# ShadowLive/ExtIO_sddc

Measured on AMD Instinct MI355X. Metric: input MSamples/s at decim=2 + achieved % HBM roofline, 1 GPU; IQ max-rel-err, higher is better.
Workload: dtype f32 (int16 in, complex64 out)

## Files before the change

extio_sddc_amd/csrc/ddc_frame_common.hpp:

```cpp
#pragma once

#include <hip/hip_runtime.h>

#include "ddc_device_io.hpp"
#include "ddc_kernels.h"
#include "fft_device.hpp"

namespace sddc {
namespace {

constexpr int NT = 256;
constexpr int HALF = 4096;
constexpr int HOP = 6144;
constexpr int BLOCK = 65536;
constexpr int FRAMES = 11;

__device__ __forceinline__ int swz(int e) { return e ^ ((e >> 4) & 15); }

template <bool RAND>
__device__ __forceinline__ float derand(int v)
{
    const float f = (float)v;
    if constexpr (!RAND) return f;
    return __int_as_float(__float_as_int(f) ^ (v << 31));
}

template <int DIR>
__device__ __forceinline__ float2 TW(float2 a, float2 w) { return DIR < 0 ? cmul(a, w) : cmulc(a, w); }

__device__ __forceinline__ float2 split_pr(float2 zk, float2 zc, float2 p, float r)
{
    const float vx = fmaf(r, zc.y, zk.x), vy = fmaf(r, zc.x, zk.y);
    return make_float2(fmaf(vx, p.x, -vy * p.y), fmaf(vx, p.y, vy * p.x));
}

template <int N>
__device__ __forceinline__ int emit_base(int k)
{
    return k == 0 ? -N / 4 : N / 2 + (3 * N / 4) * (k - 1);
}

template <int NB, bool NCO, bool CS16>
__device__ __forceinline__ void emit_frame(void *__restrict__ out, int fbase, int k, int t, const float2 (&u)[16],
                                           const OutArgs &oa, const NcoArgs &nco)
{
    const __amdgpu_buffer_rsrc_t ro = buf_rsrc(static_cast<char *>(out) + (size_t)fbase * out_bytes<CS16>());
    const int r0 = k == 0 ? 4 : 0;
#pragma unroll
    for (int r = 0; r < 12; r++) {
        if (r < r0) continue;
        float2 v = flip(u[r], oa.lsbmask);
        if constexpr (NCO) v = nco_mix(v, nco, fbase + t + NB * r);
        store_iq<CS16>(v, ro, (unsigned)t, (unsigned)(NB * r), oa);
    }
}

#define XRD(dst, expr) do { dst = (expr); asm volatile("" ::: "memory"); } while (0)

__device__ __forceinline__ void wave_lds_sync()
{
    __builtin_amdgcn_fence(__ATOMIC_RELEASE, "wavefront");
    __builtin_amdgcn_wave_barrier();
    __builtin_amdgcn_fence(__ATOMIC_ACQUIRE, "wavefront");
}

__device__ __forceinline__ void st_row(float2 *buf, unsigned A, int r, int rstride, float2 v)
{
    *(reinterpret_cast<float2 *>(reinterpret_cast<char *>(buf) + (A ^ (8u * (unsigned)r))) + rstride * r) = v;
}

__device__ __forceinline__ float2 &lds_x(float2 *buf, unsigned lane8, int R)
{
    return *reinterpret_cast<float2 *>(reinterpret_cast<char *>(buf) + (lane8 ^ (8u * (unsigned)swz(R))));
}
#define LX(buf, lane, R) lds_x(buf, 8u * (unsigned)swz(lane), R)


template <int DIR, bool EARLY>
__device__ __forceinline__ void table_twiddle(float2 *a, const float2 *tbl, int S, int j)
{
    if constexpr (EARLY) {
        float2 tw[15];
#pragma unroll
        for (int r = 1; r <= 8; r++) XRD(tw[r - 1], tbl[(r - 1) * S + j]);
#pragma unroll
        for (int r = 1; r <= 8; r++) a[r] = TW<DIR>(a[r], tw[r - 1]);
#pragma unroll
        for (int r = 9; r < 16; r++) XRD(tw[r - 1], tbl[(r - 1) * S + j]);
#pragma unroll
        for (int r = 9; r < 16; r++) a[r] = TW<DIR>(a[r], tw[r - 1]);
    } else {
#pragma unroll
        for (int r = 1; r < 16; r++) {
            float2 w;
            XRD(w, tbl[(r - 1) * S + j]);
            a[r] = TW<DIR>(a[r], w);
        }
    }
}

__device__ __forceinline__ void load_frame(const int *__restrict__ in32, int blk, int k, int (&x)[16])
{
    const __amdgpu_buffer_rsrc_t rs = buf_rsrc(in32 + ((size_t)blk * BLOCK + (size_t)k * HOP) / 2);
    const unsigned vo = 4u * threadIdx.x;
#pragma unroll
    for (int r = 0; r < 16; r++) x[r] = buf_load4<SDDC_LD_AUX>(rs, vo, 4u * NT * r);
}

}
}
```

extio_sddc_amd/csrc/ddc_fs.hip:

```cpp
#include <hip/hip_runtime.h>

#include <type_traits>

#include "ddc_frame_common.hpp"
#include "ddc_queue.hpp"
#include "ddc_stamps.hpp"
#include "ddc_fs_perm.h"
#include "split_coeffs.h"

namespace sddc {
namespace {

#ifdef SDDC_STAMPS
__device__ unsigned g_fs_stamps[2048 * 4 * kStampWords];
#endif

__device__ __forceinline__ float dpp_partner(float v)
{
    return __int_as_float(__builtin_amdgcn_mov_dpp(__float_as_int(v), 0xB1, 0xF, 0xF, true));
}

__device__ __forceinline__ void split_v2(float2 &za, float2 &vb, float2 zb, float ra, float rb)
{
    asm("s_nop 1\n\t"
        "v_fmac_f32_dpp %2, %1, %7 quad_perm:[1,0,3,2] row_mask:0xf bank_mask:0xf\n\t"
        "v_fmac_f32_dpp %3, %0, %7 quad_perm:[1,0,3,2] row_mask:0xf bank_mask:0xf\n\t"
        "v_fmac_f32_dpp %0, %5, %6 quad_perm:[1,0,3,2] row_mask:0xf bank_mask:0xf\n\t"
        "v_fmac_f32_dpp %1, %4, %6 quad_perm:[1,0,3,2] row_mask:0xf bank_mask:0xf"
        : "+v"(za.x), "+v"(za.y), "+&v"(vb.x), "+&v"(vb.y)
        : "v"(zb.x), "v"(zb.y), "v"(ra), "v"(rb));
}

__device__ __forceinline__ void split_v1(float2 &z, float2 zp, float r)
{
    asm("s_nop 1\n\t"
        "v_fmac_f32_dpp %0, %3, %4 quad_perm:[1,0,3,2] row_mask:0xf bank_mask:0xf\n\t"
        "v_fmac_f32_dpp %1, %2, %4 quad_perm:[1,0,3,2] row_mask:0xf bank_mask:0xf"
        : "+v"(z.x), "+v"(z.y)
        : "v"(zp.x), "v"(zp.y), "v"(r));
}

__device__ __forceinline__ float2 p_mul(float2 v, float2 q)
{
    return make_float2(fmaf(v.x, q.x, -v.y * q.y), fmaf(v.x, q.y, v.y * q.x));
}

template <bool LSB>
__device__ __forceinline__ float2 quarter_flip(float2 v, int s)
{
    s &= 3;
    float2 o = s == 0 ? v : s == 1 ? make_float2(v.y, -v.x) : s == 2 ? make_float2(-v.x, -v.y) : make_float2(-v.y, v.x);
    if constexpr (LSB) o.y = -o.y;
    return o;
}

template <int QT, bool LSB, bool NCO, bool CS16>
__device__ __forceinline__ void emit_frame_q(void *__restrict__ out, int fbase, int k, int t, const float2 (&u)[16],
                                             const OutArgs &oa, const NcoArgs &nco)
{
    const __amdgpu_buffer_rsrc_t ro = buf_rsrc(static_cast<char *>(out) + (size_t)fbase * out_bytes<CS16>());
    const int r0 = k == 0 ? 4 : 0;
#pragma unroll
    for (int r = 0; r < 12; r++) {
        if (r < r0) continue;
        float2 v = quarter_flip<LSB>(u[r], QT * r);
        if constexpr (NCO) v = nco_mix(v, nco, fbase + t + NT * r);
        store_iq<CS16>(v, ro, (unsigned)t, (unsigned)(NT * r), oa);
    }
}

constexpr int kQWave = 3;
constexpr int kFsPqAhead = 1;
__device__ __forceinline__ int fs_row_slot(int t) { return 272 * (t >> 4) + (t >= 128) + 34 * ((t & 15) >> 1) + (t & 1); }
__device__ __forceinline__ int fs_pair_row(int t) { return 2 * (t >> 5) + (t & 1); }
__device__ __forceinline__ int fs_pair_col(int t) { return (t >> 1) & 15; }
__device__ __forceinline__ int fs_pair_slot(int t) { return t + 2 * (t >> 5); }
constexpr int kFsLds = 4352;
constexpr int kFsTw = NT + 1;

enum { kSchedStatic = 0, kSchedQueue = 1, kSchedSteal = 2 };
template <int SCHED> struct SchedOf { using T = StealSchedule; };
template <> struct SchedOf<kSchedStatic> { using T = StaticSchedule; };
template <> struct SchedOf<kSchedQueue> { using T = FrameSchedule<1>; };

template <int ZR>
__device__ __forceinline__ constexpr bool zrow(int k) { return zr_row<ZR>(k); }

template <int SCHED, int ZR, bool RAND, bool LSB, bool NCO, bool CS16>
__global__ __launch_bounds__(NT, 4) void r2iq_fs_kernel(
    const int *__restrict__ in32, void *__restrict__ out, int nframes, const float2 *__restrict__ tw_p1,
    const float2 *__restrict__ rec_f, const float4 *__restrict__ pqf, const float2 *__restrict__ fsl, int tunebin,
    OutArgs oa, NcoArgs nco, unsigned *__restrict__ wq, int ns, unsigned slotw, int xmap, int minrem, int pub,
    unsigned *__restrict__ tlog, unsigned ttag, int use_tab, FsShares shares)
{
    __shared__ __attribute__((aligned(16))) float2 lds[kFsLds];
    __shared__ __attribute__((aligned(16))) float2 twl[15 * 16];
    __shared__ __attribute__((aligned(16))) float2 wtab[2 * kFsTw];
    __shared__ int s_next;
    static_assert(sizeof(float2) * (kFsLds + 15 * 16 + 2 * kFsTw) + sizeof(int) <= 163840 / 4,
                  "four workgroups per CU");

    const int tid = (int)threadIdx.x;
    const int w = xmap ? (int)(blockIdx.x & 7u) * (int)(gridDim.x >> 3) + (int)(blockIdx.x >> 3) : (int)blockIdx.x;
    constexpr int QLANE = 64 * kQWave;
    const bool qw = __builtin_amdgcn_readfirstlane(tid >> 6) == kQWave;
    typename SchedOf<SCHED>::T fsch;
    auto split = [&](int G, int v) __attribute__((always_inline)) {
        if constexpr (SCHED == kSchedStatic) return fs_static_split(ns, G, v, slotw, use_tab, shares);
        else return slot_split(ns, G, v, slotw);
    };
    unsigned t_start = 0u;
    if constexpr (SCHED == kSchedStatic)
        if (tlog) t_start = (unsigned)__builtin_amdgcn_s_memrealtime();
    int x[16];
    {
        const int G = (int)gridDim.x, a0 = split(G, w), b0 = split(G, w + 1);
        const int f0s = a0 < b0 ? a0 : -1;
        if (f0s >= 0) load_frame(in32, f0s / FRAMES, f0s % FRAMES, x);
        if (qw) {
            int f0[1];
            if constexpr (SCHED == kSchedSteal) fsch.init(wq, nframes, ns, w, G, slotw, f0, minrem, pub);
            else if constexpr (SCHED == kSchedStatic) fsch.init_range(a0, b0, f0);
            else fsch.init(wq, nframes, ns, w, G, slotw, f0);
            if (tid == QLANE) s_next = f0[0];
        }
        for (int i = tid; i < 15 * 16; i += NT) twl[i] = tw_p1[i];
        wtab[tid + (tid >= 128)] = rec_f[tid];
        wtab[kFsTw + tid + (tid >= 128)] = rec_f[NT + tid];
        __syncthreads();
        const int f = s_next;
        if (f >= 0 && f0s < 0) load_frame(in32, f / FRAMES, f % FRAMES, x);
    }
    int f = s_next;
    int blk = f / FRAMES, k = f - blk * FRAMES;
    const int col_ = kFsPerm[tid];
    const int qt = (tunebin >> 2) & 3;
    const bool w0 = __builtin_amdgcn_readfirstlane(tid >> 6) == 0;
    float cr[16];
    {
        const __amdgpu_buffer_rsrc_t rr = buf_rsrc(reinterpret_cast<const float *>(pqf) + 2 * HALF);
#pragma unroll
        for (int k = 0; k < 16; k++)
            if (!zrow<ZR>(k)) cr[k] = __uint_as_float(__builtin_amdgcn_raw_buffer_load_b32(rr, 4u * tid, 4u * NT * k, 0));
    }
    constexpr int AZR = ZR > 0 ? ZR : -ZR;
    constexpr int CPP = SCHED == kSchedStatic && !NCO && !CS16 && AZR >= 3 ? (AZR >= 4 && AZR <= 7 ? AZR + 1 : AZR) : 0;
    float2 cp[16];
    if constexpr (CPP > 0) {
        const __amdgpu_buffer_rsrc_t rq = buf_rsrc(pqf);
#pragma unroll
        for (int k = 0; k < 16; k++)
            if (!zrow<ZR>(k) && (k < CPP || 15 - k < CPP))
                cp[k] = buf_load8(rq, 16u * tid, 4096u * (k < 8 ? k : 15 - k) + (k < 8 ? 0u : 8u));
    }
    constexpr bool GREG = SCHED == kSchedStatic;
    float2 cg0, cg1, cg4;
    if constexpr (GREG) {
        const __amdgpu_buffer_rsrc_t rfs = buf_rsrc(fsl);
        const unsigned t8 = 8u * (unsigned)tid;
        cg0 = buf_load8(rfs, t8, 0);
        cg1 = buf_load8(rfs, t8, 8u * NT);
        cg4 = buf_load8(rfs, t8, 16u * NT);
    }
    int pA = -1, fend = -1;
    {
        const int G = (int)gridDim.x, a = split(G, w), b = split(G, w + 1);
        if constexpr (SCHED == kSchedStatic) {
            pA = b + 2;
            fend = b;
        } else if constexpr (SCHED == kSchedSteal) {
            const int len = b - a, two = len < 2 ? len : 2;
            pA = minrem <= 0 ? b + 2 : a + (pub > 0 && len - pub > two ? len - pub : two);
            fend = minrem <= 0 ? b : pA;
        }
    }
    ST_INIT();

    auto frame = [&](auto phase) __attribute__((always_inline)) {
        constexpr bool PB = decltype(phase)::value;
        if constexpr (PB && SCHED != kSchedSteal)
            if (qw) fsch.peek();
        int z = 0;
        asm volatile("" : "+s"(z));
        const int t = tid + z;
        const int c = col_ + z;
        const int oblk = blk * 8 * HALF;
        const int kc = k;
        float2 v[16];
        {
            float2 a[16];
#pragma unroll
            for (int r = 0; r < 16; r++)
                if constexpr (RAND) {
                    const int wd = x[r] ^ (int)(((unsigned)x[r] & 0x10001u) * 0xFFFEu);
                    a[r] = make_float2((float)(int)(short)(wd & 0xffff), (float)(wd >> 16));
                } else {
                    a[r] = make_float2((float)(int)(short)(x[r] & 0xffff), (float)(x[r] >> 16));
                }
            dft16<-1>(a, v);
        }
        {
            float2 *const row = lds + fs_row_slot(t);
#pragma unroll
            for (int r = 0; r < 16; r++) row[2 * r] = v[r];
        }
        ST_SYNC(1);
        {
            float2 a[16];
            const float2 *const col = lds + fs_pair_slot(t);
#pragma unroll
            for (int r = 0; r < 16; r++) XRD(a[r], col[272 * r + (r >= 8)]);
            table_twiddle<-1, true>(a, twl, 16, fs_pair_col(t));
            dft16<-1>(a, v);
        }
        {
            float2 *const col = lds + fs_pair_slot(t);
#pragma unroll
            for (int r = 0; r < 16; r++) col[272 * r + (r >= 8)] = v[r];
        }
        ST_SYNC(3);
        if constexpr (PB && SCHED == kSchedSteal)
            if (qw) fsch.peek();
        const __amdgpu_buffer_rsrc_t rpq = buf_rsrc(pqf + z);
        const unsigned t16 = 16u * (unsigned)t;
        float2 qa[8], qb[8];
        constexpr bool P16 = ZR != 2 && ZR != -2 && SCHED != kSchedSteal;
        auto pload = [&](int p) __attribute__((always_inline)) {
            const bool za = zrow<ZR>(p), zb = zrow<ZR>(15 - p);
            if (p < CPP) {
                if (!za) qa[p] = cp[p];
                if (!zb) qb[p] = cp[15 - p];
            } else if (!za && !zb && !P16) {
                qa[p] = buf_load8(rpq, t16, 4096u * p);
                qb[p] = buf_load8(rpq, t16, 4096u * p + 8u);
            } else if (!za && !zb) {
                const float4 q = buf_load16(rpq, t16, 4096u * p);
                qa[p] = make_float2(q.x, q.y);
                qb[p] = make_float2(q.z, q.w);
            } else if (!za) {
                qa[p] = buf_load8(rpq, t16, 4096u * p);
            } else if (!zb) {
                qb[p] = buf_load8(rpq, t16, 4096u * p + 8u);
            }
        };
#pragma unroll
        for (int p = 0; p < kFsPqAhead; p++) {
            pload(p);
        }
        asm volatile("" ::: "memory");
        {
            float2 a[16];
            const float2 *const cb = lds + 272 * (c >> 4) + (c >= 128) + 2 * (c & 15);
#pragma unroll
            for (int r = 0; r < 16; r++) XRD(a[r], cb[34 * (r >> 1) + (r & 1)]);
            const int cw = c + (c >= 128);
            const float2 fw1 = wtab[cw], fw4 = wtab[kFsTw + cw];
            twiddle_rec16<-1>(a, fw1, fw4);
            dft16<-1>(a, v);
        }
        float2 u[16];
        {
            float2 a[16];
            auto split_w0 = [&]() __attribute__((always_inline)) {
                const int lane = t & 63;
#pragma unroll
                for (int p = 0; p < 8; p++) {
                    if (p + kFsPqAhead < 8) {
                        const int pn = p + kFsPqAhead;
                        pload(pn);
                        asm volatile("" ::: "memory");
                    }
#pragma unroll
                    for (int h = 0; h < 2; h++) {
                        const int kk = h ? 15 - p : p;
                        if (zrow<ZR>(kk)) continue;
                        const float2 q = h ? qb[p] : qa[p];
                        const float2 vm = v[15 - kk], v0m = v[(16 - kk) & 15];
                        float2 zc = make_float2(dpp_partner(vm.x), dpp_partner(vm.y));
                        zc = lane == 1 ? vm : zc;
                        zc = lane == 0 ? v0m : zc;
                        float2 vv = make_float2(fmaf(cr[kk], zc.y, v[kk].x), fmaf(cr[kk], zc.x, v[kk].y));
                        if (kk == 8) vv = lane == 0 ? make_float2(v[8].x, -v[8].y) : vv;
                        a[kk] = p_mul(vv, q);
                    }
                }
            };
            auto split_generic = [&]() __attribute__((always_inline)) {
#pragma unroll
                for (int p = 0; p < 8; p++) {
                    if (p + kFsPqAhead < 8) {
                        const int pn = p + kFsPqAhead;
                        pload(pn);
                        asm volatile("" ::: "memory");
                    }
                    if (zrow<ZR>(15 - p)) {
                        split_v1(v[p], v[15 - p], cr[p]);
                        a[p] = p_mul(v[p], qa[p]);
                    } else if (zrow<ZR>(p)) {
                        split_v1(v[15 - p], v[p], cr[15 - p]);
                        a[15 - p] = p_mul(v[15 - p], qb[p]);
                    } else {
                        float2 vb = v[15 - p];
                        split_v2(v[p], vb, v[15 - p], cr[p], cr[15 - p]);
                        a[p] = p_mul(v[p], qa[p]);
                        a[15 - p] = p_mul(vb, qb[p]);
                    }
                }
            };
            if constexpr (ZR != 0) {
                int wv = __builtin_amdgcn_readfirstlane(t >> 6);
                asm volatile("" : "+s"(wv));
                if (w0) split_w0();
                if (wv != 0) split_generic();
            } else {
                if (w0) split_w0();
                else split_generic();
            }
            dft16z<+1, ZR>(a, u);
        }
        {
            int c1 = c;
            asm volatile("" : "+v"(c1));
            float2 *const cb = lds + 272 * (c1 >> 4) + (c1 >= 128) + 2 * (c1 & 15);
#pragma unroll
            for (int r = 0; r < 16; r++) cb[34 * (r >> 1) + (r & 1)] = u[r];
        }
        if constexpr (PB) {
            if (qw) {
                const int f_n = fsch.next();
                if (tid == QLANE) s_next = f_n;
            }
        }
        ST_SYNC(5);
        const __amdgpu_buffer_rsrc_t rfs = buf_rsrc(fsl);
        const unsigned t8 = 8u * (unsigned)t;
        float2 g0, g1, g4;
        if constexpr (GREG) {
            g0 = cg0;
            g1 = cg1;
            g4 = cg4;
        } else {
            g0 = buf_load8(rfs, t8, 0);
            g1 = buf_load8(rfs, t8, 8u * NT);
            g4 = buf_load8(rfs, t8, 16u * NT);
        }
        int fn;
        {
            float2 a[16];
            const float2 *const ib = lds + fs_pair_slot(t);
#pragma unroll
            for (int r = 0; r < 16; r++) XRD(a[r], ib[272 * r + (r >= 8)]);
            if constexpr (PB) fn = s_next;
            else fn = f + 1 < fend ? f + 1 : -1;
            if (fn >= 0) {
                blk = fn / FRAMES;
                k = fn - blk * FRAMES;
                load_frame(in32, blk, k, x);
            }
            if constexpr (PB)
                if (qw) fsch.take();
            table_twiddle<+1, true>(a, twl, 16, fs_pair_row(t));
            dft16<+1>(a, u);
        }
        {
            int t1 = t;
            asm volatile("" : "+v"(t1));
            float2 *const ib = lds + fs_pair_slot(t1);
#pragma unroll
            for (int r = 0; r < 16; r++) ib[272 * r + (r >= 8)] = u[r];
        }
        ST_SYNC(7);
        {
            float2 a[16];
            const float2 *const rb = lds + fs_row_slot(t);
#pragma unroll
            for (int r = 0; r < 16; r++) XRD(a[r], rb[2 * r]);
            const int tw = t + (t >= 128);
            const float2 rw1 = wtab[tw], rw4 = wtab[kFsTw + tw];
            twiddle_g16<+1>(a, g0, g1, g4, rw1, rw4);
            dft16<+1>(a, u);
            const int fb = oblk + emit_base<HALF>(kc);
            switch (qt) {
            case 0: emit_frame_q<0, LSB, NCO, CS16>(out, fb, kc, t, u, oa, nco); break;
            case 1: emit_frame_q<1, LSB, NCO, CS16>(out, fb, kc, t, u, oa, nco); break;
            case 2: emit_frame_q<2, LSB, NCO, CS16>(out, fb, kc, t, u, oa, nco); break;
            default: emit_frame_q<3, LSB, NCO, CS16>(out, fb, kc, t, u, oa, nco); break;
            }
        }
        if constexpr (SCHED == kSchedSteal) {
            if constexpr (PB)
                if (qw) fsch.take_late();
        }
        ST_FRAME_END();
        f = fn;
    };
    if constexpr (SCHED != kSchedQueue)
        while (f >= 0 && f + 2 < pA) frame(std::false_type{});
    if constexpr (SCHED != kSchedStatic) {
        if constexpr (SCHED == kSchedSteal)
            if (qw) fsch.enter(f);
        while (f >= 0) frame(std::true_type{});
    }
    ST_WRITE(g_fs_stamps, w, tid);
    if constexpr (SCHED == kSchedStatic) {
        if (tlog && tid == 0) {
            const unsigned t_end = (unsigned)__builtin_amdgcn_s_memrealtime();
            reinterpret_cast<uint4 *>(tlog)[w] = make_uint4(t_start, t_end, ttag, t_start ^ t_end ^ ttag);
        }
    }
    if constexpr (SCHED == kSchedQueue)
        if (tid == QLANE) fs_queue_done(wq, (unsigned)gridDim.x);
}

__global__ void build_fs_tables_kernel(const float2 *__restrict__ hsel0, const float2 *__restrict__ tw4096,
                                       int tunebin, float4 *__restrict__ pqf, float2 *__restrict__ fsl)
{
    const int i = (int)(blockIdx.x * blockDim.x + threadIdx.x);
    if (i >= HALF) return;
    const int l = i & (NT - 1), kk = i >> 8;
    const int b = kFsPerm[l] + NT * kk;
    const bool band = (b >= tunebin && b - tunebin < HALF / 2) || (b < tunebin && tunebin - b <= HALF / 2);
    float3 c = make_float3(0.f, 0.f, 0.f);
    if (band) {
        const int m = (b - tunebin) & (HALF - 1);
        const SplitCoeffs k = split_pr_coeffs(hsel0[m].x, hsel0[m].y, b, kSplitQ0);
        c = make_float3(k.px, k.py, k.r);
    }
    reinterpret_cast<float2 *>(pqf)[2 * (NT * (kk < 8 ? kk : 15 - kk) + l) + (kk >= 8)] = make_float2(c.x, c.y);
    reinterpret_cast<float *>(pqf)[2 * HALF + i] = c.z;
    if (i < NT) {
        fsl[i] = tw4096[(tunebin * i) & (HALF - 1)];
        fsl[NT + i] = tw4096[((tunebin - 1) * i) & (HALF - 1)];
        fsl[2 * NT + i] = tw4096[((tunebin - 4) * i) & (HALF - 1)];
    }
}

template <int SCHED, int ZR, bool RAND, bool LSB, bool NCO, bool CS16>
hipError_t launch_fs_s(const KernelTables &t, const int16_t *d_in, int nblk, void *d_out, const float4 *pqf,
                       const float2 *fsl, int tunebin, const OutArgs &oa, const NcoArgs &nco, unsigned *wq,
                       const FsSched &fs, int device, hipStream_t s)
{
    auto kern = r2iq_fs_kernel<SCHED, ZR, RAND, LSB, NCO, CS16>;
    const int static_pct = SCHED == kSchedQueue ? fs.static_pct : 100, fpw = fs.fpw;
    int occ = 0, cus = 0;
    hipError_t e = launch_geometry(t.lc, reinterpret_cast<const void *>(kern), NT, device, &occ, &cus);
    if (e != hipSuccess) return e;
    const int nframes = nblk * FRAMES;
    int grid = cus * occ;
    if (grid > nframes) grid = nframes;
    int ns = frame_schedule_static(nframes, static_pct);
    unsigned slotw = occ == 4 && grid == cus * occ ? (fs.slotw ? fs.slotw : kFsSlotWeights) : 0u;
    const FsShares *tab = nullptr;
    unsigned *tlog = nullptr, ttag = 0u;
    if (SCHED == kSchedStatic && fs.adapt && slotw != 0u && fs.slotw == 0u && fpw <= 0 && grid <= kFsShareMaxG &&
        !fs.adapt(fs.adapt_ctx, grid, ns, &tab, &tlog, &ttag)) {
        tab = nullptr;
        tlog = nullptr;
    }
    static const FsShares kNoShares = {};
    int xmap = 0;
    if (fpw > 0) {
        grid = (nframes + fpw - 1) / fpw;
        ns = nframes;
        slotw = 0u;
        xmap = (grid & 7) == 0 && grid * fpw == nframes;
    }
    int minrem = fs.minrem;
    if (SCHED == kSchedSteal && (grid > kFsStealMax || 2LL * nframes / grid + 1 > kStealMaxRange)) minrem = 0;
    hipLaunchKernelGGL(kern, dim3((unsigned)grid), dim3(NT), 0, s, reinterpret_cast<const int *>(d_in), d_out, nframes,
// ... 105 lines not shown
```

extio_sddc_amd/csrc/ddc_runtime.cpp:

```cpp
#include <hip/hip_runtime_api.h>

#include <algorithm>
#include <cmath>
#include <complex>
#include <cstdarg>
#include <cstdio>
#include <cstdlib>
#include <cstring>
#include <memory>
#include <mutex>
#include <new>
#include <string>
#include <type_traits>
#include <vector>

#include "cpu/r2iq_cpu.h"
#include "ddc_kernels.h"
#include "filterbank.h"
#include "fine_tune.h"
#include "fs_split_controller.hpp"
#include "sddc_fft.h"
#include "sddc_ddc.h"
#include "sddc_ddc_internal.h"

namespace {

thread_local std::string g_last_error;

int fail(int code, const char *fmt, ...)
{
    char buf[512];
    va_list ap;
    va_start(ap, fmt);
    vsnprintf(buf, sizeof buf, fmt, ap);
    va_end(ap);
    g_last_error = buf;
    return code;
}

#define HIP_TRY(expr)                                                                         \
    do {                                                                                      \
        hipError_t e_ = (expr);                                                               \
        if (e_ != hipSuccess)                                                                 \
            return fail(SDDC_ERR_HIP, "%s failed: %s (%s:%d)", #expr, hipGetErrorString(e_),  \
                        __FILE__, __LINE__);                                                  \
    } while (0)

struct DeviceGuard {
    int prev = -1;
    hipError_t err = hipSuccess;
    explicit DeviceGuard(int dev)
    {
        if (hipGetDevice(&prev) != hipSuccess) prev = -1;
        if (prev != dev) err = hipSetDevice(dev);
    }
    ~DeviceGuard()
    {
        int cur = -1;
        if (prev >= 0 && hipGetDevice(&cur) == hipSuccess && cur != prev) (void)hipSetDevice(prev);
    }
};

constexpr int kHistory = SDDC_DDC_HALF_FFT;
constexpr int kBlock = SDDC_DDC_BLOCK;
constexpr int kHostChunk = 32;
constexpr size_t kOutBlockMax = (size_t)SDDC_DDC_OUT_BLOCK * 2 * sizeof(float);
constexpr size_t kChNcoBlockBytes = (size_t)SDDC_DDC_OUT_BLOCK / sddc::FineTune::kBlock * sddc::FineTune::kLanes * sizeof(float2);
constexpr size_t kChNcoTableCap = (size_t)128 << 20;
static_assert(kChNcoBlockBytes == 8192, "4 lane starts per 128 output samples");
static_assert(SDDC_DDC_MAX_CHANNELS * kChNcoBlockBytes <= kChNcoTableCap, "one block of every channel fits the cap");

struct Readers {
    std::vector<std::pair<hipStream_t, hipEvent_t>> v;

    hipError_t record(hipStream_t s)
    {
        for (auto &p : v)
            if (p.first == s) return hipEventRecord(p.second, s);
        if (v.size() >= 16) {
            hipError_t e = sync();
            if (e != hipSuccess) return e;
            clear();
        }
        hipEvent_t ev = nullptr;
        hipError_t e = hipEventCreateWithFlags(&ev, hipEventDisableTiming);
        if (e != hipSuccess) return e;
        v.emplace_back(s, ev);
        return hipEventRecord(ev, s);
    }
    hipError_t order_before(hipStream_t s) const
    {
        for (const auto &p : v)
            if (p.first != s) {
                hipError_t e = hipStreamWaitEvent(s, p.second, 0);
                if (e != hipSuccess) return e;
            }
        return hipSuccess;
    }
    hipError_t order_after(hipStream_t other, hipStream_t s) const
    {
        if (other == s) return hipSuccess;
        for (const auto &p : v)
            if (p.first == other) return hipStreamWaitEvent(s, p.second, 0);
        return hipSuccess;
    }
    hipError_t sync() const
    {
        for (const auto &p : v) {
            hipError_t e = hipEventSynchronize(p.second);
            if (e != hipSuccess) return e;
        }
        return hipSuccess;
    }
    void clear()
    {
        for (auto &p : v) (void)hipEventDestroy(p.second);
        v.clear();
    }
};

struct ChannelStream {
    std::vector<float> taps;
    int nch = 0, H = 0;
    float *d_taps = nullptr;
    size_t taps_cap = 0;
    float2 *d_tail[2] = {};
    int cur = 0;
    std::vector<float> tail_h;
    Readers readers;
    int max_wgs = 0;
    void *d_in = nullptr;
    float *d_out = nullptr;
    size_t in_cap = 0, out_cap = 0;

    void clear()
    {
        taps.clear();
        nch = H = 0;
        tail_h.clear();
        for (float2 *&p : d_tail) {
            if (p) (void)hipFree(p);
            p = nullptr;
        }
        cur = 0;
    }
    void free_all()
    {
        clear();
        if (d_taps) (void)hipFree(d_taps);
        if (d_in) (void)hipFree(d_in);
        if (d_out) (void)hipFree(d_out);
        d_taps = nullptr;
        d_in = nullptr;
        d_out = nullptr;
        taps_cap = in_cap = out_cap = 0;
        readers.clear();
    }
    int configure(sddc_ddc *h, const char *name, const float *t, int ntaps, const float *ordered, size_t nordered,
                  int H_, int nch_);
    int reset(sddc_ddc *h);
    template <class F> int launch(hipStream_t s, F fn)
    {
        HIP_TRY(readers.order_before(s));
        const hipError_t e = fn(d_tail[cur], d_tail[cur ^ 1]);
        const hipError_t er = readers.record(s);
        HIP_TRY(e);
        if (H > 0) cur ^= 1;
        HIP_TRY(er);
        return SDDC_OK;
    }
};

struct ChannelDemod {
    std::vector<sddc::ChDemChannel> chan;
    int nch = 0, out_fmt = 0;
    uint32_t pos = 0;
    sddc::ChDemChannel *d_chan = nullptr;
    float2 *d_last[2] = {};
    int cur = 0;
    std::vector<float> last_h;
    float *d_partial = nullptr;
    size_t partial_cap = 0;
    Readers readers;
    int max_wgs = 0;
    void *d_in = nullptr, *d_out = nullptr;
    float *d_pow = nullptr;
    size_t in_cap = 0, out_cap = 0, pow_cap = 0;

    void clear()
    {
        chan.clear();
        nch = out_fmt = 0;
        pos = 0;
        last_h.clear();
        if (d_chan) (void)hipFree(d_chan);
// ... 102 lines not shown
        d_in = d_out = nullptr;
        scratch_cap = in_cap = out_cap = env_cap = 0;
        readers.clear();
    }
};

}

struct sddc_ddc {
    int device = 0;
    float gain = 0.f;
    int d = 0, lsb = 0, rand = 0, tunebin = SDDC_DDC_HALF_FFT / 4;
    int out_fmt = SDDC_DDC_FMT_CF32;
    float cs16_scale = 1.f;
    sddc::KernelTables tables;
    sddc::LaunchCache launch_cache;
    float2 *d_tables = nullptr;

    mutable std::mutex mu;
    hipStream_t stream = nullptr;

    struct HostSlot {
        int16_t *d_in = nullptr;
        void *d_out = nullptr;
        int16_t *h_in = nullptr;
        void *h_out = nullptr;
        hipEvent_t e_h2d = nullptr, e_k = nullptr, e_d2h = nullptr;
    } hs[2];
    hipStream_t s_in = nullptr, s_out = nullptr;
    bool host_ready = false;
    int last_slot = -1, last_n = 0;
    std::vector<std::pair<const char *, size_t>> regions;

    int *d_tunebins = nullptr;
    std::vector<int> tunebins_cached;
    int2 *d_windows = nullptr;
    int windows_d = -1;
    float2 *d_chscratch = nullptr;
    int chscratch_rows = 0;
    Readers ch_readers;

    float4 *d_pq = nullptr;
    int pq_d = -1, pq_tb = -1;
    hipStream_t pq_s = nullptr;
    float4 *d_fs = nullptr;
    int fs_tb = -1;
    hipStream_t fs_s = nullptr;
    static constexpr int kQueueSlots = 64;
    unsigned *d_queue = nullptr;
    int queue_slot = 0;
    int slot_weights = sddc::kSlotWeighting;
    sddc::FsSched fs_sched;
    hipStream_t q_s[kQueueSlots] = {};

    struct FsAdapt {
        static constexpr int kRing = 16;
        static constexpr int kTaint = 4;
        static constexpr int kEager = 32;
        static constexpr int kEvery = 8;
        bool on = true;
        sddc::FsSplitController ctl;
        std::vector<float> forced;
        unsigned *h_ring = nullptr, *d_ring = nullptr;
        bool ring_failed = false;
        struct Pending {
            unsigned tag = 0u;
            int G = 0, ns = 0;
            bool live = false, tainted = false;
            std::vector<int> n;
        } pend[kRing];
        int next = 0, last_pending = -1;
        unsigned seq = 0u;
        sddc::FsShares tab = {};
        std::vector<int> tab_n, base_n;
        int tab_ns = -1, base_ns = -1;
        hipStream_t cur_s = nullptr, last_s = nullptr;
        bool have_last = false;
        int taint_left = 0;
        long launches = 0, skipped = 0;
        int last_table = 0, last_logged = 0;
    } fsa;
    bool q_used[kQueueSlots] = {};
    bool q_dirty[kQueueSlots] = {};
    Readers readers;

    float nco_fc = 0.f;
    sddc::FineTune nco;
    static constexpr int kNcoSlots = 3;
    float2 *h_nco[kNcoSlots] = {};
    hipEvent_t nco_ev[kNcoSlots] = {};
    size_t h_nco_cap = 0;
    int nco_slot = 0;
    float2 *d_nco = nullptr;
    size_t d_nco_cap = 0;

    std::vector<float> chnco_fc;
    float2 *d_chnco_trig = nullptr;
    float2 *d_chnco_state = nullptr;
    float *d_chnco_fc = nullptr;
    float2 *d_chnco_starts = nullptr;
    size_t chnco_starts_cap = 0;
    int chnco_run_blocks = 0;

    std::vector<int16_t> hist_override;

    std::vector<float> sp_win;
    double sp_wsum = (double)SDDC_DDC_FFTN;
    float *d_sp_win = nullptr;
    float *d_sp_partial = nullptr;
    size_t sp_partial_cap = 0;
    int16_t *d_sp_in = nullptr;
    float *d_sp_out = nullptr;
    size_t sp_host_cap = 0;
    Readers sp_readers;
    int sp_max_wgs = 0;

    std::vector<float> chsp_win;
    int chsp_n = 0;
    double chsp_wsum = 0.0;
    float *d_chsp_win = nullptr;
    void *d_chsp_in = nullptr;
    float *d_chsp_out = nullptr;
    size_t chsp_in_cap = 0, chsp_out_cap = 0;
    Readers chsp_readers;
    int chsp_max_wgs = 0;

    ChannelStream chdec, chres;
    int chdec_R = 0;
    int chres_L = 0, chres_M = 0, chres_e = 0;
    ChannelDemod chdem;
    ChannelAudio chaud;
    ChannelAgc chagc;

    std::unique_ptr<sddc::cpu::R2iq> cpu;

    long inject_fail = -1;
    long inject_late = -1;
};

static int tuning_of(float offset, float *delta)
{
    const int tb = (int)(offset * SDDC_DDC_HALF_FFT / 4) * 4;
    *delta = ((float)tb / SDDC_DDC_HALF_FFT) - offset;
    return std::min(std::max(tb, 0), SDDC_DDC_HALF_FFT - 4);
}

static bool injected_failure(sddc_ddc_t *h)
{
    if (h->inject_fail < 0) return false;
    return h->inject_fail-- == 0;
}
static bool injected_late_failure(sddc_ddc_t *h)
{
    if (h->inject_late < 0) return false;
    return h->inject_late-- == 0;
}

template <class T>
static int grow_device_buffer(T **ptr, size_t *cap, size_t need, const char *who, const char *what)
{
    if (need <= *cap) return SDDC_OK;
    if (*ptr) (void)hipFree(*ptr);
    *ptr = nullptr;
    *cap = 0;
    constexpr size_t elem = sizeof(std::conditional_t<std::is_void<T>::value, char, T>);
    if (hipMalloc(ptr, need * elem) != hipSuccess) {
        (void)hipGetLastError();
// ... 710 lines not shown

int sddc_ddc_set_channel_fine_tune(sddc_ddc_t *h, const float *relative_freqs, int nch)
{
    using sddc::FineTune;
    if (!h) return fail(SDDC_ERR_ARG, "null handle");
    if (nch < 0 || nch > SDDC_DDC_MAX_CHANNELS)
        return fail(SDDC_ERR_ARG, "channel fine tune: channel count %d outside 0..%d", nch, SDDC_DDC_MAX_CHANNELS);
    if (!relative_freqs) nch = 0;
    for (int c = 0; c < nch; c++)
        if (!std::isfinite(relative_freqs[c]))
            return fail(SDDC_ERR_ARG, "channel fine tune: non-finite frequency of channel %d", c);
    std::lock_guard<std::mutex> lk(h->mu);
    if (h->cpu) return fail(SDDC_ERR_STATE, "channel fine tune: a CPU handle has no many-channel path");
    if (nch == 0) {
        h->chnco_fc.clear();
        return SDDC_OK;
    }
    const bool all = h->chnco_fc.size() != (size_t)nch;
    std::vector<char> changed((size_t)nch);
    bool any = false;
    for (int c = 0; c < nch; c++) any |= (changed[c] = all || relative_freqs[c] != h->chnco_fc[c]) != 0;
    if (!any) return SDDC_OK;
    DeviceGuard g(h->device);
    HIP_TRY(g.err);
    HIP_TRY(h->ch_readers.sync());
    if (!h->d_chnco_trig) HIP_TRY(hipMalloc(&h->d_chnco_trig, SDDC_DDC_MAX_CHANNELS * FineTune::kTable * sizeof(float2)));
    if (!h->d_chnco_state) HIP_TRY(hipMalloc(&h->d_chnco_state, SDDC_DDC_MAX_CHANNELS * FineTune::kLanes * sizeof(float2)));
    if (!h->d_chnco_fc) HIP_TRY(hipMalloc(&h->d_chnco_fc, SDDC_DDC_MAX_CHANNELS * sizeof(float)));
    h->chnco_fc.clear();
    std::vector<float2> trig((size_t)nch * FineTune::kTable), state((size_t)nch * FineTune::kLanes);
    for (int c = 0; c < nch; c++) {
        if (!changed[c]) continue;
        FineTune ft;
        ft.init(relative_freqs[c], 0.0f);
        std::memcpy(&trig[(size_t)c * FineTune::kTable], ft.table(), FineTune::kTable * sizeof(float2));
        ft.starts(1, &state[(size_t)c * FineTune::kLanes]);
    }
    for (int c0 = 0; c0 < nch;) {
        if (!changed[c0]) {
            c0++;
            continue;
        }
        int c1 = c0 + 1;
        while (c1 < nch && changed[c1]) c1++;
        const size_t n = (size_t)(c1 - c0);
        HIP_TRY(hipMemcpy(h->d_chnco_trig + (size_t)c0 * FineTune::kTable, &trig[(size_t)c0 * FineTune::kTable],
                          n * FineTune::kTable * sizeof(float2), hipMemcpyHostToDevice));
        HIP_TRY(hipMemcpy(h->d_chnco_state + (size_t)c0 * FineTune::kLanes, &state[(size_t)c0 * FineTune::kLanes],
                          n * FineTune::kLanes * sizeof(float2), hipMemcpyHostToDevice));
        HIP_TRY(hipMemcpy(h->d_chnco_fc + c0, relative_freqs + c0, n * sizeof(float), hipMemcpyHostToDevice));
        c0 = c1;
    }
    h->chnco_fc.assign(relative_freqs, relative_freqs + nch);
    return SDDC_OK;
}

int sddc_ddc_internal_set_param(sddc_ddc_t *h, int param, int value)
{
    if (!h) return fail(SDDC_ERR_ARG, "null handle");
    std::lock_guard<std::mutex> lk(h->mu);
    switch (param) {
    case SDDC_DDC_PARAM_SLOT_WEIGHTS:
        h->slot_weights = value != 0;
        return SDDC_OK;
    case SDDC_DDC_PARAM_FS_STATIC_PCT:
        if (value < 0 || value > 100) return fail(SDDC_ERR_ARG, "static share %d outside 0..100", value);
        h->fs_sched.static_pct = value;
        return SDDC_OK;
    case SDDC_DDC_PARAM_FS_FRAMES_PER_WG:
        if (value < 0 || value > 1024) return fail(SDDC_ERR_ARG, "frames per workgroup %d outside 0..1024", value);
        h->fs_sched.fpw = value;
        return SDDC_OK;
    case SDDC_DDC_PARAM_FS_SCHEDULE:
        if (value < 0 || value > 2) return fail(SDDC_ERR_ARG, "FS schedule %d outside 0..2", value);
        h->fs_sched.sched = value;
        return SDDC_OK;
    case SDDC_DDC_PARAM_FS_STEAL_MINREM:
        if (value < 0 || value > 64) return fail(SDDC_ERR_ARG, "steal threshold %d outside 0..64", value);
        h->fs_sched.minrem = value;
        return SDDC_OK;
    case SDDC_DDC_PARAM_FS_ZERO_ROWS:
        h->fs_sched.zr = value != 0;
        return SDDC_OK;
    case SDDC_DDC_PARAM_FS_SLOT_WEIGHTS: {
        for (int k = 0; k < 4 && value != 0; k++) {
            const int wk = (value >> (8 * k)) & 0xff;
            if (wk < 1 || wk > 127) return fail(SDDC_ERR_ARG, "slot weight %d of slot %d outside 1..127", wk, k);
        }
        h->fs_sched.slotw = (unsigned)value;
        return SDDC_OK;
    }
    case SDDC_DDC_PARAM_FS_STEAL_PUBLIC:
        if (value < 0 || value > 1024) return fail(SDDC_ERR_ARG, "public frames %d outside 0..1024", value);
        h->fs_sched.pub = value;
        return SDDC_OK;
    case SDDC_DDC_PARAM_FS_ADAPTIVE_SPLIT:
        h->fsa.on = value != 0;
        return SDDC_OK;
    case SDDC_DDC_PARAM_CH_NCO_RUN_BLOCKS:
        if (value < 0 || value > SDDC_DDC_MAX_BLOCKS)
            return fail(SDDC_ERR_ARG, "run blocks %d outside 0..%d", value, SDDC_DDC_MAX_BLOCKS);
        h->chnco_run_blocks = value;
        return SDDC_OK;
    case SDDC_DDC_PARAM_SPECTRUM_MAX_WGS:
        if (value < 0) return fail(SDDC_ERR_ARG, "spectrum workgroup cap %d is negative", value);
        h->sp_max_wgs = value;
        return SDDC_OK;
    case SDDC_DDC_PARAM_CHSPEC_MAX_WGS:
        if (value < 0) return fail(SDDC_ERR_ARG, "channel spectrum workgroup cap %d is negative", value);
        h->chsp_max_wgs = value;
        return SDDC_OK;
    case SDDC_DDC_PARAM_CHDEC_MAX_WGS:
        if (value < 0) return fail(SDDC_ERR_ARG, "channel decimator workgroup cap %d is negative", value);
        h->chdec.max_wgs = value;
        return SDDC_OK;
    case SDDC_DDC_PARAM_CHRES_MAX_WGS:
        if (value < 0) return fail(SDDC_ERR_ARG, "channel resampler workgroup cap %d is negative", value);
        h->chres.max_wgs = value;
        return SDDC_OK;
    case SDDC_DDC_PARAM_CHDEM_MAX_WGS:
        if (value < 0) return fail(SDDC_ERR_ARG, "channel demodulator workgroup cap %d is negative", value);
        h->chdem.max_wgs = value;
        return SDDC_OK;
    case SDDC_DDC_PARAM_CHAUD_MAX_WGS:
        if (value < 0) return fail(SDDC_ERR_ARG, "channel audio filter workgroup cap %d is negative", value);
        h->chaud.max_wgs = value;
        return SDDC_OK;
    case SDDC_DDC_PARAM_CHAUD_RUN_BLOCKS:
        if (value < 0 || value > (1 << 20))
            return fail(SDDC_ERR_ARG, "channel audio filter run length %d outside 0..2^20 blocks", value);
        h->chaud.run_blocks = value;
        return SDDC_OK;
    case SDDC_DDC_PARAM_CHAGC_MAX_WGS:
        if (value < 0) return fail(SDDC_ERR_ARG, "channel AGC workgroup cap %d is negative", value);
        h->chagc.max_wgs = value;
        return SDDC_OK;
    case SDDC_DDC_PARAM_CHAGC_RUN_BLOCKS:
        if (value < 0 || value > (1 << 20))
            return fail(SDDC_ERR_ARG, "channel AGC run length %d outside 0..2^20 blocks", value);
        h->chagc.run_blocks = value;
        return SDDC_OK;
    default:
        return fail(SDDC_ERR_ARG, "unknown parameter %d", param);
    }
}

int sddc_ddc_internal_fs_set_shares(sddc_ddc_t *h, const float *shares, int n)
{
    if (!h) return fail(SDDC_ERR_ARG, "null handle");
    if (n < 0 || n > sddc::kFsShareMaxG || (n > 0 && !shares)) return fail(SDDC_ERR_ARG, "shares: n %d outside 0..%d", n, sddc::kFsShareMaxG);
    double sum = 0.0;
    for (int w = 0; w < n; w++) {
        if (!(shares[w] >= 0.f) || !std::isfinite(shares[w])) return fail(SDDC_ERR_ARG, "share %d is negative or not finite", w);
        sum += shares[w];
    }
    if (n > 0 && !(sum > 0.0)) return fail(SDDC_ERR_ARG, "shares: all zero");
    std::lock_guard<std::mutex> lk(h->mu);
    h->fsa.forced.assign(shares, shares + n);
    if (h->fsa.ctl.forced()) h->fsa.ctl.unload();
    h->fsa.tab_ns = -1;
    return SDDC_OK;
}

int sddc_ddc_internal_fs_split_state(sddc_ddc_t *h, long *info, int *counts, int ncounts)
{
    if (!h) return fail(SDDC_ERR_ARG, "null handle");
// ... 1673 lines not shown
```

extio_sddc_amd/csrc/sddc_ddc_internal.h:

```cpp
#pragma once
#include "sddc_ddc.h"
#ifdef __cplusplus
extern "C" {
#endif
#define SDDC_DDC_PARAM_FS_STATIC_PCT 1
#define SDDC_DDC_PARAM_SLOT_WEIGHTS 2
#define SDDC_DDC_PARAM_FS_FRAMES_PER_WG 3
#define SDDC_DDC_PARAM_FS_SCHEDULE 4
#define SDDC_DDC_PARAM_FS_STEAL_MINREM 5
#define SDDC_DDC_PARAM_FS_STEAL_PUBLIC 6
#define SDDC_DDC_PARAM_FS_ZERO_ROWS 7
#define SDDC_DDC_PARAM_FS_SLOT_WEIGHTS 8
#define SDDC_DDC_PARAM_CH_NCO_RUN_BLOCKS 9
#define SDDC_DDC_PARAM_FS_ADAPTIVE_SPLIT 10
#define SDDC_DDC_PARAM_SPECTRUM_MAX_WGS 11
#define SDDC_DDC_PARAM_CHSPEC_MAX_WGS 12
#define SDDC_DDC_PARAM_CHDEC_MAX_WGS 13
#define SDDC_DDC_PARAM_CHRES_MAX_WGS 14

#define SDDC_DDC_PARAM_CHDEM_MAX_WGS 15

#define SDDC_DDC_PARAM_CHAUD_MAX_WGS 16

#define SDDC_DDC_PARAM_CHAUD_RUN_BLOCKS 17

#define SDDC_DDC_PARAM_CHAGC_MAX_WGS 18

#define SDDC_DDC_PARAM_CHAGC_RUN_BLOCKS 19

int sddc_ddc_internal_set_param(sddc_ddc_t *h, int param, int value);
int sddc_ddc_internal_fs_set_shares(sddc_ddc_t *h, const float *shares, int n);
int sddc_ddc_internal_fs_split_state(sddc_ddc_t *h, long *info, int *counts, int ncounts);
int sddc_ddc_internal_chdec_layout(int factor, int ntaps, int cs16, int *tile, int *pitch, int *store_conflicts);
int sddc_ddc_internal_chres_layout(int up, int down, int ntaps, int cs16, int *tile_outputs, int *pitch,
                                   int *store_conflicts);
int sddc_ddc_internal_chres_set_position(sddc_ddc_t *h, uint64_t pos);
int sddc_ddc_internal_chdem_set_position(sddc_ddc_t *h, uint32_t pos);
int sddc_ddc_internal_chaud_set_position(sddc_ddc_t *h, uint64_t pos);
int sddc_ddc_internal_chagc_set_position(sddc_ddc_t *h, uint64_t pos);
int sddc_ddc_internal_demod_angle(const float *im, const float *re, size_t n, float *out);
int sddc_ddc_internal_demod_sincos(const uint32_t *words, size_t n, float *c, float *s);
void *sddc_fs_split_create(int G, unsigned slot_weights);
void sddc_fs_split_destroy(void *c);
int sddc_fs_split_load(void *c, const float *shares, int n);
int sddc_fs_split_table(void *c, int ns, unsigned *p, int *first);
int sddc_fs_split_update(void *c, const int *n, const unsigned *start, const unsigned *end);
int sddc_fs_split_model(void *c, double *cost, double *offset);
int sddc_ddc_internal_fs_stamps(unsigned *host, int nwords, int *words_per_wave);
int sddc_ddc_internal_p_stamps(unsigned *host, int nwords, int *words_per_wave);
#ifdef __cplusplus
}
#endif
```

Baseline: 666,500.

## Pack per-thread LDS base addresses into four registers and defer reader event records

In the static-schedule FS kernel, per-thread LDS row, column and twiddle base addresses are precomputed once and packed as 16-bit pairs into four VGPRs. Opaque asm keeps the compiler from rematerialising them, which is meant to cut repeated address arithmetic and register pressure. Separately, reader event recording on the host is made lazy by default: hipEventRecord is deferred until some consumer needs the event, saving API calls per launch. The packing depends on the LDS footprint fitting 16-bit addresses, and lazy recording changes when events are placed on streams.

```diff
diff --git a/extio_sddc_amd/csrc/ddc_frame_common.hpp b/extio_sddc_amd/csrc/ddc_frame_common.hpp
--- a/extio_sddc_amd/csrc/ddc_frame_common.hpp
+++ b/extio_sddc_amd/csrc/ddc_frame_common.hpp
@@ -99,12 +99,15 @@
     }
 }
 
+__device__ __forceinline__ void load_frame(const int *__restrict__ in32, int blk, int k, int (&x)[16], unsigned vo)
+{
+    const __amdgpu_buffer_rsrc_t rs = buf_rsrc(in32 + ((size_t)blk * BLOCK + (size_t)k * HOP) / 2);
+#pragma unroll
+    for (int r = 0; r < 16; r++) x[r] = buf_load4<SDDC_LD_AUX>(rs, vo, 4u * NT * r);
+}
 __device__ __forceinline__ void load_frame(const int *__restrict__ in32, int blk, int k, int (&x)[16])
 {
-    const __amdgpu_buffer_rsrc_t rs = buf_rsrc(in32 + ((size_t)blk * BLOCK + (size_t)k * HOP) / 2);
-    const unsigned vo = 4u * threadIdx.x;
-#pragma unroll
-    for (int r = 0; r < 16; r++) x[r] = buf_load4<SDDC_LD_AUX>(rs, vo, 4u * NT * r);
+    load_frame(in32, blk, k, x, 4u * threadIdx.x);
 }
 
 }
diff --git a/extio_sddc_amd/csrc/ddc_fs.hip b/extio_sddc_amd/csrc/ddc_fs.hip
--- a/extio_sddc_amd/csrc/ddc_fs.hip
+++ b/extio_sddc_amd/csrc/ddc_fs.hip
@@ -6,7 +6,12 @@
 #include "ddc_queue.hpp"
 #include "ddc_stamps.hpp"
 #include "ddc_fs_perm.h"
+#include "fs_bases.h"
 #include "split_coeffs.h"
+
+#ifndef SDDC_FS_RECOMPUTED
+#define SDDC_FS_RECOMPUTED 0
+#endif
 
 namespace sddc {
 namespace {
@@ -40,6 +45,19 @@
         : "v"(zp.x), "v"(zp.y), "v"(r));
 }
 
+typedef __attribute__((address_space(3))) float2 lds_float2;
+__device__ __forceinline__ unsigned lds_addr(const float2 *p)
+{
+    return (unsigned)(size_t)(const lds_float2 *)p;
+}
+#if defined(__HIP_DEVICE_COMPILE__)
+__device__ __forceinline__ float2 *lds_at(unsigned a) { return (float2 *)(lds_float2 *)a; }
+#else
+__device__ __forceinline__ float2 *lds_at(unsigned) { return nullptr; }
+#endif
+
+__device__ __forceinline__ void fs_opaque(unsigned &w) { asm volatile("" : "+v"(w)); }
+
 __device__ __forceinline__ float2 p_mul(float2 v, float2 q)
 {
     return make_float2(fmaf(v.x, q.x, -v.y * q.y), fmaf(v.x, q.y, v.y * q.x));
@@ -71,12 +89,7 @@
 
 constexpr int kQWave = 3;
 constexpr int kFsPqAhead = 1;
-__device__ __forceinline__ int fs_row_slot(int t) { return 272 * (t >> 4) + (t >= 128) + 34 * ((t & 15) >> 1) + (t & 1); }
-__device__ __forceinline__ int fs_pair_row(int t) { return 2 * (t >> 5) + (t & 1); }
-__device__ __forceinline__ int fs_pair_col(int t) { return (t >> 1) & 15; }
-__device__ __forceinline__ int fs_pair_slot(int t) { return t + 2 * (t >> 5); }
-constexpr int kFsLds = 4352;
-constexpr int kFsTw = NT + 1;
+static_assert(kFsTw == NT + 1 && kFsTwl == 15 * 16, "fs_bases.h");
 
 enum { kSchedStatic = 0, kSchedQueue = 1, kSchedSteal = 2 };
 template <int SCHED> struct SchedOf { using T = StealSchedule; };
@@ -133,9 +146,20 @@
     }
     int f = s_next;
     int blk = f / FRAMES, k = f - blk * FRAMES;
+    constexpr bool PK = SCHED == kSchedStatic && SDDC_FS_RECOMPUTED == 0;
+    static_assert(sizeof(float2) * (kFsLds + kFsTwl + 2 * kFsTw) + sizeof(int) <= 65536, "fs_bases.h: 16-bit LDS addresses");
     const int col_ = kFsPerm[tid];
+    unsigned b0 = 0u, b1 = 0u, b2 = 0u, b3 = 0u;
+    if constexpr (PK) {
+        const FsBases fb = fs_bases_pack(tid, col_, lds_addr(lds), lds_addr(twl), lds_addr(wtab));
+        b0 = fb.p[0];
+        b1 = fb.p[1];
+        b2 = fb.p[2];
+        b3 = fb.p[3];
+    }
     const int qt = (tunebin >> 2) & 3;
     const bool w0 = __builtin_amdgcn_readfirstlane(tid >> 6) == 0;
+    const int widx = __builtin_amdgcn_readfirstlane(tid >> 6);
     float cr[16];
     {
         const __amdgpu_buffer_rsrc_t rr = buf_rsrc(reinterpret_cast<const float *>(pqf) + 2 * HALF);
@@ -182,8 +206,8 @@
             if (qw) fsch.peek();
         int z = 0;
         asm volatile("" : "+s"(z));
-        const int t = tid + z;
-        const int c = col_ + z;
+        const int t = PK ? 0 : tid + z;
+        const int c = PK ? 0 : col_ + z;
         const int oblk = blk * 8 * HALF;
         const int kc = k;
         float2 v[16];
@@ -200,21 +224,44 @@
             dft16<-1>(a, v);
         }
         {
-            float2 *const row = lds + fs_row_slot(t);
+            float2 *row;
+            if constexpr (PK) {
+                fs_opaque(b0);
+                row = lds_at(fs_lo(b0));
+            } else {
+                row = lds + fs_row_slot(t);
+            }
 #pragma unroll
             for (int r = 0; r < 16; r++) row[2 * r] = v[r];
         }
         ST_SYNC(1);
         {
             float2 a[16];
-            const float2 *const col = lds + fs_pair_slot(t);
+            const float2 *col;
+            if constexpr (PK) {
+                fs_opaque(b0);
+                col = lds_at(fs_hi(b0));
+            } else {
+                col = lds + fs_pair_slot(t);
+            }
 #pragma unroll
             for (int r = 0; r < 16; r++) XRD(a[r], col[272 * r + (r >= 8)]);
-            table_twiddle<-1, true>(a, twl, 16, fs_pair_col(t));
+            if constexpr (PK) {
+                fs_opaque(b2);
+                table_twiddle<-1, true>(a, lds_at(fs_hi(b2)), 16, 0);
+            } else {
+                table_twiddle<-1, true>(a, twl, 16, fs_pair_col(t));
+            }
             dft16<-1>(a, v);
         }
         {
-            float2 *const col = lds + fs_pair_slot(t);
+            float2 *col;
+            if constexpr (PK) {
+                fs_opaque(b0);
+                col = lds_at(fs_hi(b0));
+            } else {
+                col = lds + fs_pair_slot(t);
+            }
 #pragma unroll
             for (int r = 0; r < 16; r++) col[272 * r + (r >= 8)] = v[r];
         }
@@ -222,7 +269,13 @@
         if constexpr (PB && SCHED == kSchedSteal)
             if (qw) fsch.peek();
         const __amdgpu_buffer_rsrc_t rpq = buf_rsrc(pqf + z);
-        const unsigned t16 = 16u * (unsigned)t;
+        unsigned t16;
+        if constexpr (PK) {
+            fs_opaque(b3);
+            t16 = fs_t16(b3);
+        } else {
+            t16 = 16u * (unsigned)t;
+        }
         float2 qa[8], qb[8];
         constexpr bool P16 = ZR != 2 && ZR != -2 && SCHED != kSchedSteal;
         auto pload = [&](int p) __attribute__((always_inline)) {
@@ -250,11 +303,22 @@
         asm volatile("" ::: "memory");
         {
             float2 a[16];
-            const float2 *const cb = lds + 272 * (c >> 4) + (c >= 128) + 2 * (c & 15);
+            const float2 *cb, *wc;
+            if constexpr (PK) {
+                fs_opaque(b1);
+                cb = lds_at(fs_lo(b1));
+            } else {
+                cb = lds + fs_col_slot(c);
+            }
 #pragma unroll
             for (int r = 0; r < 16; r++) XRD(a[r], cb[34 * (r >> 1) + (r & 1)]);
-            const int cw = c + (c >= 128);
-            const float2 fw1 = wtab[cw], fw4 = wtab[kFsTw + cw];
+            if constexpr (PK) {
+                fs_opaque(b1);
+                wc = lds_at(fs_hi(b1));
+            } else {
+                wc = wtab + fs_tw_slot(c);
+            }
+            const float2 fw1 = wc[0], fw4 = wc[kFsTw];
             twiddle_rec16<-1>(a, fw1, fw4);
             dft16<-1>(a, v);
         }
@@ -262,7 +326,13 @@
         {
             float2 a[16];
             auto split_w0 = [&]() __attribute__((always_inline)) {
-                const int lane = t & 63;
+                int lane;
+                if constexpr (PK) {
+                    fs_opaque(b3);
+                    lane = (int)fs_lane(b3);
+                } else {
+                    lane = t & 63;
+                }
 #pragma unroll
                 for (int p = 0; p < 8; p++) {
                     if (p + kFsPqAhead < 8) {
@@ -308,7 +378,7 @@
                 }
             };
             if constexpr (ZR != 0) {
-                int wv = __builtin_amdgcn_readfirstlane(t >> 6);
+                int wv = PK ? widx : __builtin_amdgcn_readfirstlane(t >> 6);
                 asm volatile("" : "+s"(wv));
                 if (w0) split_w0();
                 if (wv != 0) split_generic();
@@ -321,7 +391,13 @@
         {
             int c1 = c;
             asm volatile("" : "+v"(c1));
-            float2 *const cb = lds + 272 * (c1 >> 4) + (c1 >= 128) + 2 * (c1 & 15);
+            float2 *cb;
+            if constexpr (PK) {
+                fs_opaque(b1);
+                cb = lds_at(fs_lo(b1));
+            } else {
+                cb = lds + fs_col_slot(c1);
+            }
 #pragma unroll
             for (int r = 0; r < 16; r++) cb[34 * (r >> 1) + (r & 1)] = u[r];
         }
@@ -347,7 +423,13 @@
         int fn;
         {
             float2 a[16];
-            const float2 *const ib = lds + fs_pair_slot(t);
+            const float2 *ib;
+            if constexpr (PK) {
+                fs_opaque(b0);
+                ib = lds_at(fs_hi(b0));
+            } else {
+                ib = lds + fs_pair_slot(t);
+            }
 #pragma unroll
             for (int r = 0; r < 16; r++) XRD(a[r], ib[272 * r + (r >= 8)]);
             if constexpr (PB) fn = s_next;
@@ -355,36 +437,68 @@
             if (fn >= 0) {
                 blk = fn / FRAMES;
                 k = fn - blk * FRAMES;
-                load_frame(in32, blk, k, x);
+                if constexpr (PK) {
+                    fs_opaque(b3);
+                    load_frame(in32, blk, k, x, fs_t4(b3));
+                } else {
+                    load_frame(in32, blk, k, x);
+                }
             }
             if constexpr (PB)
                 if (qw) fsch.take();
-            table_twiddle<+1, true>(a, twl, 16, fs_pair_row(t));
+            if constexpr (PK) {
+                fs_opaque(b3);
+                table_twiddle<+1, true>(a, lds_at(fs_lo(b3)), 16, 0);
+            } else {
+                table_twiddle<+1, true>(a, twl, 16, fs_pair_row(t));
+            }
             dft16<+1>(a, u);
         }
         {
             int t1 = t;
             asm volatile("" : "+v"(t1));
-            float2 *const ib = lds + fs_pair_slot(t1);
+            float2 *ib;
+            if constexpr (PK) {
+                fs_opaque(b0);
+                ib = lds_at(fs_hi(b0));
+            } else {
+                ib = lds + fs_pair_slot(t1);
+            }
 #pragma unroll
             for (int r = 0; r < 16; r++) ib[272 * r + (r >= 8)] = u[r];
         }
         ST_SYNC(7);
         {
             float2 a[16];
-            const float2 *const rb = lds + fs_row_slot(t);
+            const float2 *rb, *wt;
+            if constexpr (PK) {
+                fs_opaque(b0);
+                rb = lds_at(fs_lo(b0));
+            } else {
+                rb = lds + fs_row_slot(t);
+            }
 #pragma unroll
             for (int r = 0; r < 16; r++) XRD(a[r], rb[2 * r]);
-            const int tw = t + (t >= 128);
-            const float2 rw1 = wtab[tw], rw4 = wtab[kFsTw + tw];
+            if constexpr (PK) {
+                fs_opaque(b2);
+                wt = lds_at(fs_lo(b2));
+            } else {
+                wt = wtab + fs_tw_slot(t);
+            }
+            const float2 rw1 = wt[0], rw4 = wt[kFsTw];
             twiddle_g16<+1>(a, g0, g1, g4, rw1, rw4);
             dft16<+1>(a, u);
             const int fb = oblk + emit_base<HALF>(kc);
+            int te = t;
+            if constexpr (PK) {
+                fs_opaque(b3);
+                te = (int)fs_t(b3);
+            }
             switch (qt) {
-            case 0: emit_frame_q<0, LSB, NCO, CS16>(out, fb, kc, t, u, oa, nco); break;
-            case 1: emit_frame_q<1, LSB, NCO, CS16>(out, fb, kc, t, u, oa, nco); break;
-            case 2: emit_frame_q<2, LSB, NCO, CS16>(out, fb, kc, t, u, oa, nco); break;
-            default: emit_frame_q<3, LSB, NCO, CS16>(out, fb, kc, t, u, oa, nco); break;
+            case 0: emit_frame_q<0, LSB, NCO, CS16>(out, fb, kc, te, u, oa, nco); break;
+            case 1: emit_frame_q<1, LSB, NCO, CS16>(out, fb, kc, te, u, oa, nco); break;
+            case 2: emit_frame_q<2, LSB, NCO, CS16>(out, fb, kc, te, u, oa, nco); break;
+            default: emit_frame_q<3, LSB, NCO, CS16>(out, fb, kc, te, u, oa, nco); break;
             }
         }
         if constexpr (SCHED == kSchedSteal) {
diff --git a/extio_sddc_amd/csrc/ddc_runtime.cpp b/extio_sddc_amd/csrc/ddc_runtime.cpp
--- a/extio_sddc_amd/csrc/ddc_runtime.cpp
+++ b/extio_sddc_amd/csrc/ddc_runtime.cpp
@@ -71,12 +71,21 @@
 static_assert(SDDC_DDC_MAX_CHANNELS * kChNcoBlockBytes <= kChNcoTableCap, "one block of every channel fits the cap");
 
 struct Readers {
-    std::vector<std::pair<hipStream_t, hipEvent_t>> v;
+    struct Entry {
+        hipStream_t first;
+        hipEvent_t second;
+        bool pending;
+    };
+    std::vector<Entry> v;
+    bool lazy = false;
 
     hipError_t record(hipStream_t s)
     {
         for (auto &p : v)
-            if (p.first == s) return hipEventRecord(p.second, s);
+            if (p.first == s) {
+                p.pending = true;
+                return lazy ? hipSuccess : flush(p);
+            }
         if (v.size() >= 16) {
             hipError_t e = sync();
             if (e != hipSuccess) return e;
@@ -85,32 +94,46 @@
         hipEvent_t ev = nullptr;
         hipError_t e = hipEventCreateWithFlags(&ev, hipEventDisableTiming);
         if (e != hipSuccess) return e;
-        v.emplace_back(s, ev);
-        return hipEventRecord(ev, s);
-    }
-    hipError_t order_before(hipStream_t s) const
+        v.push_back(Entry{s, ev, true});
+        return lazy ? hipSuccess : flush(v.back());
+    }
+    static hipError_t flush(Entry &p)
     {
-        for (const auto &p : v)
+        if (!p.pending) return hipSuccess;
+        hipError_t e = hipEventRecord(p.second, p.first);
+        if (e == hipSuccess) p.pending = false;
+        return e;
+    }
+    hipError_t order_before(hipStream_t s)
+    {
+        for (auto &p : v)
             if (p.first != s) {
-                hipError_t e = hipStreamWaitEvent(s, p.second, 0);
+                hipError_t e = flush(p);
+                if (e == hipSuccess) e = hipStreamWaitEvent(s, p.second, 0);
                 if (e != hipSuccess) return e;
             }
         return hipSuccess;
     }
-    hipError_t order_after(hipStream_t other, hipStream_t s) const
+    hipError_t order_after(hipStream_t other, hipStream_t s)
     {
         if (other == s) return hipSuccess;
-        for (const auto &p : v)
-            if (p.first == other) return hipStreamWaitEvent(s, p.second, 0);
+        for (auto &p : v)
+            if (p.first == other) {
+                hipError_t e = flush(p);
+                return e == hipSuccess ? hipStreamWaitEvent(s, p.second, 0) : e;
+            }
         return hipSuccess;
     }
-    hipError_t sync() const
+    hipError_t sync()
     {
-        for (const auto &p : v) {
-            hipError_t e = hipEventSynchronize(p.second);
-            if (e != hipSuccess) return e;
-        }
-        return hipSuccess;
+        hipError_t first = hipSuccess;
+        for (auto &p : v) {
+            hipError_t e = flush(p);
+            const hipError_t es = hipEventSynchronize(p.second);
+            if (e == hipSuccess) e = es;
+            if (e != hipSuccess && first == hipSuccess) first = e;
+        }
+        return first;
     }
     void clear()
     {
@@ -379,7 +402,7 @@
     } fsa;
     bool q_used[kQueueSlots] = {};
     bool q_dirty[kQueueSlots] = {};
-    Readers readers;
+    Readers readers{{}, true};
 
     float nco_fc = 0.f;
     sddc::FineTune nco;
@@ -1256,6 +1279,9 @@
     case SDDC_DDC_PARAM_FS_ZERO_ROWS:
         h->fs_sched.zr = value != 0;
         return SDDC_OK;
+    case SDDC_DDC_PARAM_LAZY_RECORD:
+        h->readers.lazy = value != 0;
+        return SDDC_OK;
     case SDDC_DDC_PARAM_FS_SLOT_WEIGHTS: {
         for (int k = 0; k < 4 && value != 0; k++) {
             const int wk = (value >> (8 * k)) & 0xff;
diff --git a/extio_sddc_amd/csrc/fs_bases.h b/extio_sddc_amd/csrc/fs_bases.h
--- /dev/null
+++ b/extio_sddc_amd/csrc/fs_bases.h
@@ -0,0 +1,47 @@
+#pragma once
+
+#include <stdint.h>
+
+#ifndef SDDC_HD
+#if defined(__HIPCC__)
+#define SDDC_HD __host__ __device__
+#else
+#define SDDC_HD
+#endif
+#endif
+
+namespace sddc {
+
+SDDC_HD inline int fs_row_slot(int t) { return 272 * (t >> 4) + (t >= 128) + 34 * ((t & 15) >> 1) + (t & 1); }
+SDDC_HD inline int fs_pair_row(int t) { return 2 * (t >> 5) + (t & 1); }
+SDDC_HD inline int fs_pair_col(int t) { return (t >> 1) & 15; }
+SDDC_HD inline int fs_pair_slot(int t) { return t + 2 * (t >> 5); }
+SDDC_HD inline int fs_col_slot(int c) { return 272 * (c >> 4) + (c >= 128) + 2 * (c & 15); }
+SDDC_HD inline int fs_tw_slot(int j) { return j + (j >= 128); }
+
+constexpr int kFsLds = 4352;
+constexpr int kFsTw = 256 + 1;
+constexpr int kFsTwl = 15 * 16;
+
+struct FsBases {
+    uint32_t p[4];
+};
+
+SDDC_HD inline FsBases fs_bases_pack(int t, int c, uint32_t lds0, uint32_t twl0, uint32_t wtab0)
+{
+    FsBases b;
+    b.p[0] = (lds0 + 8u * (uint32_t)fs_row_slot(t)) | (lds0 + 8u * (uint32_t)fs_pair_slot(t)) << 16;
+    b.p[1] = (lds0 + 8u * (uint32_t)fs_col_slot(c)) | (wtab0 + 8u * (uint32_t)fs_tw_slot(c)) << 16;
+    b.p[2] = (wtab0 + 8u * (uint32_t)fs_tw_slot(t)) | (twl0 + 8u * (uint32_t)fs_pair_col(t)) << 16;
+    b.p[3] = (twl0 + 8u * (uint32_t)fs_pair_row(t)) | (16u * (uint32_t)t) << 16;
+    return b;
+}
+
+SDDC_HD inline uint32_t fs_lo(uint32_t w) { return w & 0xffffu; }
+SDDC_HD inline uint32_t fs_hi(uint32_t w) { return w >> 16; }
+SDDC_HD inline uint32_t fs_t16(uint32_t w) { return w >> 16; }
+SDDC_HD inline uint32_t fs_t4(uint32_t w) { return w >> 18; }
+SDDC_HD inline uint32_t fs_t(uint32_t w) { return w >> 20; }
+SDDC_HD inline uint32_t fs_lane(uint32_t w) { return (w >> 20) & 63u; }
+
+}
diff --git a/extio_sddc_amd/csrc/sddc_ddc_internal.h b/extio_sddc_amd/csrc/sddc_ddc_internal.h
--- a/extio_sddc_amd/csrc/sddc_ddc_internal.h
+++ b/extio_sddc_amd/csrc/sddc_ddc_internal.h
@@ -28,6 +28,8 @@
 
 #define SDDC_DDC_PARAM_CHAGC_RUN_BLOCKS 19
 
+#define SDDC_DDC_PARAM_LAZY_RECORD 20
+
 int sddc_ddc_internal_set_param(sddc_ddc_t *h, int param, int value);
 int sddc_ddc_internal_fs_set_shares(sddc_ddc_t *h, const float *shares, int n);
 int sddc_ddc_internal_fs_split_state(sddc_ddc_t *h, long *info, int *counts, int ncounts);
```

Result: faster. 678,000, median of 6 (+1.7%).
